# webster-781/DyGLib

Hardware: AMD Instinct MI355X
Metric: edges/sec (link-prediction fwd) DyGFormer Wikipedia (higher is better)
Workload: dtype f32; 1 GPU; DyGFormer link-prediction forward, synthetic wikipedia-shaped graph (8227+1000 nodes, 157474 edges), L=64, P=2, batch=200, 2 layers, 2 heads, C=50; pos+neg calls + MergeLayer+sigmoid per step; batch=200, max_input_sequence_length=64, patch_size=2, parallelism=1 x edge-batch shard, graph+weights replicated, metric all-reduce over RCCL, impl=auto, streams=1, steps_per_launch=32

## Files before the change

### dyglib_amd/_build.py

```python
from __future__ import annotations

import concurrent.futures as cf
import hashlib
import os
import shutil
import subprocess
import sys
from typing import List

CSRC = os.path.join(os.path.dirname(os.path.abspath(__file__)), "csrc")
INCLUDE = os.path.join(os.path.dirname(os.path.dirname(os.path.abspath(__file__))), "include")
LIB_NAME = "libdygnn_hip.so"
LIB_PATH = os.path.join(CSRC, LIB_NAME)
SOURCES = ["csr_host.cpp", "sampler.hip", "cooccurrence.hip", "dygformer_generic.hip", "dygformer_fused3.hip", "dygformer_fused3_train.hip",
           "dygformer_fused3_bwd.hip", "dygformer_fused3_pack.hip", "dygformer_pack_plan.hip", "dygformer_pooled_tail.hip", "dygformer_proj_tables.hip", "dygformer_train.hip",
           "dygformer_api.hip", "gemm.hip", "tgat.hip", "tgat_chain.hip", "tgat_train.hip", "tgn.hip", "tgn_train.hip", "graphmixer.hip", "graphmixer_train.hip", "tcl.hip", "tcl_train.hip", "cawn.hip",
           "cawn_train.hip", "metrics.hip", "edgebank.hip", "memory_rnn.hip"]
ARCH = "gfx950"
CXXFLAGS = ["-O3", "-std=c++17", "-fPIC", f"--offload-arch={ARCH}", "-Wall", "-Wno-unused-function",
            "-ffp-contract=off"]


SANITIZE = ["-fsanitize=address,undefined", "-fno-omit-frame-pointer", "-g", "-shared-libsan", "-Wno-option-ignored"]
VARIANTS = {"": [], "stamps": ["-DDYGNN_STAMPS=1"], "asan": SANITIZE}
for _k, _v in list(os.environ.items()):
    if _k.startswith("DYGNN_VARIANT_"):
        VARIANTS[_k[len("DYGNN_VARIANT_"):].lower()] = _v.split()
LINK_EXTRA = {"asan": ["-fsanitize=address,undefined", "-shared-libsan"]}


def asan_runtime() -> str:
    import glob
    hits = glob.glob("/opt/rocm/lib/llvm/lib/clang/*/lib/linux/libclang_rt.asan-x86_64.so")
    if not hits:
        raise RuntimeError("libclang_rt.asan-x86_64.so not found under /opt/rocm/lib/llvm")
    return hits[0]


def lib_path(variant: str = "") -> str:
    return LIB_PATH if not variant else os.path.join(CSRC, f"libdygnn_hip_{variant}.so")


def _hipcc() -> str:
    for cand in (os.environ.get("HIPCC"), "/opt/rocm/bin/hipcc", shutil.which("hipcc")):
        if cand and os.path.exists(cand):
            return cand
    raise RuntimeError("hipcc not found (looked at $HIPCC, /opt/rocm/bin/hipcc, PATH)")

# ... 67 lines not shown
```

### dyglib_amd/csrc/common.h

```cpp
#pragma once
#include <hip/hip_runtime.h>
#include <cstdarg>
#include <cstdint>
#include <cstdio>

#include "../../include/dygnn.h"

namespace dygnn {

void set_error(const char* fmt, ...);

inline hipStream_t as_stream(dygnn_stream_t s) { return reinterpret_cast<hipStream_t>(s); }

constexpr int kWave = 64;

inline int64_t ceil_div(int64_t a, int64_t b) { return (a + b - 1) / b; }

struct Carve {
    size_t o = 0;
    size_t take(size_t bytes) { const size_t r = o; o += (bytes + 255) & ~size_t(255); return r; }
};

__device__ __forceinline__ int64_t wave_lower_bound(const double* __restrict__ ts, int64_t lo, int64_t hi, double t, int lane) {
    while (hi - lo > kWave) {
        const int64_t step = (hi - lo + kWave - 1) / kWave;
        const int64_t p = lo + (int64_t)lane * step;
        const bool pred = (p < hi) && (ts[p] < t);
        const int c = __popcll(__ballot(pred));
        if (c == 0) return lo;
        const int64_t nlo = lo + (int64_t)(c - 1) * step + 1;
        const int64_t nhi = lo + (int64_t)c * step;
        hi = nhi < hi ? nhi : hi;
        lo = nlo;
    }
    const int64_t p = lo + lane;
    const bool pred = (p < hi) && (ts[p] < t);
    return lo + __popcll(__ballot(pred));
}

}

#define DYGNN_REQUIRE(cond, ...)                                  \
    do {                                                          \
        if (!(cond)) {                                            \
            dygnn::set_error(__VA_ARGS__);                        \
            return DYGNN_E_INVALID;                               \
        }                                                         \
    } while (0)

#define DYGNN_HIP(expr)                                                                        \
    do {                                                                                       \
        hipError_t _e = (expr);                                                                \
        if (_e != hipSuccess) {                                                                \
            dygnn::set_error("%s failed: %s (%s:%d)", #expr, hipGetErrorString(_e), __FILE__, __LINE__); \
            return DYGNN_E_HIP;                                                                \
        }                                                                                      \
    } while (0)

#define DYGNN_LAUNCH_CHECK() DYGNN_HIP(hipGetLastError())
```

### dyglib_amd/csrc/dygformer_fused3.hip

```cpp
#include "fused3_forward.h"

namespace dygnn {

namespace v3 {
__global__ __launch_bounds__(512, 2) void k_dygformer_fused3_packed(const Args a) {
    fused3_body<4, false, 8, 3, true>(a);
}
}

static void drop_zero_channels(v3::Args& a, uint32_t table_flags) {
    using namespace v3;
    const int node_frags = 4 * proj_slots(a.nchunk[0]), time_frags = 4 * proj_slots(a.nchunk[2]), edge_frags = 4 * proj_slots(a.nchunk[1]);
    if (table_flags & DYGNN_TABLE_NODE_ZERO) { a.proj_skip0 = node_frags; a.proj_frags -= node_frags; a.nchunk[0] = 0; }
    a.proj_cut = (a.nchunk[0] ? node_frags : 0) + time_frags;
    if (table_flags & DYGNN_TABLE_EDGE_ZERO) { a.proj_skip1 = edge_frags; a.proj_frags -= edge_frags; a.nchunk[1] = 0; }
}

int forward_fused3(const Dims& d, const PackedLayout& pl, const dygnn_dygformer_weights* w, const float* packed,
                   const dygnn_csr* csr, const float* node_feat, const float* edge_feat, const int64_t* src,
                   const int64_t* dst, const double* times, int64_t B, int64_t G, int64_t pair_stride, float* out_src, float* out_dst, char* ws,
                   const WorkspaceLayout& wl, const dygnn_dygformer_taps* taps, uint32_t table_flags, const float* node_proj, const float* edge_proj,
                   hipStream_t s) {
    using namespace v3;
    if (!supported(d)) { set_error("fused kernel: unsupported shape"); return DYGNN_E_UNSUPPORTED; }
    if (int rc = window_lengths_device(d, csr, src, dst, times, B, G, ws, wl, s)) return rc;
    Args a{};
    PackLayout3 f;
    if (int rc = fused3_args(d, pl, w, packed, csr, node_feat, edge_feat, src, dst, times, B, G, out_src, out_dst, ws, wl, taps, a, f)) return rc;
    if (table_flags & DYGNN_TABLE_NODE_ZERO) node_proj = nullptr;
    if (table_flags & DYGNN_TABLE_EDGE_ZERO) edge_proj = nullptr;
    drop_zero_channels(a, table_flags | (node_proj ? DYGNN_TABLE_NODE_ZERO : 0u) | (edge_proj ? DYGNN_TABLE_EDGE_ZERO : 0u));
    a.pt_node = node_proj; a.pt_edge = edge_proj;
    if (taps && taps->seq_lens) DYGNN_HIP(hipMemcpyAsync(taps->seq_lens, ws + wl.dims + 2 * sizeof(int32_t), 2 * sizeof(int32_t), hipMemcpyDeviceToDevice, s));
    if (taps && taps->ev_kernel_start) DYGNN_HIP(hipEventRecord(static_cast<hipEvent_t>(taps->ev_kernel_start), s));
    a.pair_stride = (f.np == 2 && pair_stride > 0) ? pair_stride : 0;
    const bool tap_last = taps && taps->layer_out[d.NL - 1] != nullptr;
    if (!tap_last) { a.stream = packed + pl.fused3 + f.stream_p; a.nstages = f.nstages_p; }
    bool untapped = !tap_last && !(taps && (taps->encoder_input || taps->phase_cycles));
    for (int l = 0; l < d.NL; ++l) untapped = untapped && !(taps && taps->layer_out[l]);
    const int pk_env = pack_pairs_env();
    const size_t plan_off = plan_offset(B, G);
    const bool pack_ok = untapped && f.np == 2 && f.scr_floats8 > 0 && B <= INT32_MAX && plan_off > 0 && pk_env != 0;
    const bool small = f.np == 2 && a.pair_stride == 0 && B <= kSmallBatchPairs && !small_off() && !(pack_ok && pk_env == 1);
    const unsigned grid = small || f.np != 2 ? (unsigned)B : (unsigned)(a.pair_stride ? a.pair_stride : (B + 1) / 2);
    auto launch = [&](auto kern, unsigned threads) -> int {
        DYGNN_HIP(hipFuncSetAttribute(reinterpret_cast<const void*>(kern), hipFuncAttributeMaxDynamicSharedMemorySize, kLdsBytes));
        hipLaunchKernelGGL(kern, dim3(grid), dim3(threads), kLdsBytes, s, a);
        return DYGNN_OK;
    };
    const bool tail = !tap_last && (pooled_tail_wanted(grid) || (pack_ok && pk_env == 1));
    const bool pack_it = pack_ok && !small && tail;
    int rc;
    if (pack_it) {
        if (int rcp = pack_plan_device(d, B, G, ws, wl, s)) return rcp;
        a.plan = reinterpret_cast<const int32_t*>(ws + wl.dims + plan_off);
        a.pair_stride = 0; a.scr_floats = f.scr_floats8; a.slab_chunks = f.slab_chunks8; a.tab_off = 0; a.tab_slots = 0; a.tab_bits = 0;
        rc = launch(k_dygformer_fused3_packed, 512);
    } else if (tail) rc = small ? launch(k_dygformer_fused3<4, false, 4, 3>, 256) : f.np == 2 ? launch(k_dygformer_fused3<4, false, 8, 3>, 512) : launch(k_dygformer_fused3<8, false, 8, 3>, 512);
    else if (small) rc = tap_last ? launch(k_dygformer_fused3<4, false, 4, 2>, 256) : launch(k_dygformer_fused3<4, false, 4, 1>, 256);
    else if (f.np == 2) rc = tap_last ? launch(k_dygformer_fused3<4, false, 8, 2>, 512) : launch(k_dygformer_fused3<4, false, 8, 1>, 512);
    else rc = tap_last ? launch(k_dygformer_fused3<8, false, 8, 2>, 512) : launch(k_dygformer_fused3<8, false, 8, 1>, 512);
    if (rc) return rc;
    DYGNN_LAUNCH_CHECK();
    if (tail)
        if (int rc2 = pooled_tail(a.pooled_rows, 2 * B, a.w2frag, a.b2_last, a.outfrag, a.outb, a.Fn, out_src, out_dst, s)) return rc2;
    if (taps && taps->ev_kernel_stop) DYGNN_HIP(hipEventRecord(static_cast<hipEvent_t>(taps->ev_kernel_stop), s));
    return DYGNN_OK;
}

}
```

### dyglib_amd/csrc/dygformer_pack_plan.hip

```cpp
#include "dygformer_layout.h"
#include "fused3_plan.h"

namespace dygnn {
namespace v3 {

constexpr int kPlanThreads = 1024;

__device__ __forceinline__ int pair_tile_count(const int32_t* hist_len, const CallDims* cd, int64_t b, int64_t B, int64_t G, int L, int P) {
    const CallDims d = cd[b / G];
    const PairTokens t = pair_tokens(hist_len[b], hist_len[B + b], L, P, d.T_s, d.T_d);
    const int nt = (t.Tc + 15) / 16;
    return nt < 1 ? 1 : nt > 4 ? 4 : nt;
}

__global__ __launch_bounds__(kPlanThreads) void k_pack_plan(const int32_t* hist_len, const CallDims* cd, int64_t B, int64_t G, int L, int P, int32_t* plan,
                                                            int32_t max_wg) {
    __shared__ int32_t cnt[2][4][kPlanThreads];
    __shared__ PackPlan pp;
    const int t = threadIdx.x;
    const int64_t chunk = (B + kPlanThreads - 1) / kPlanThreads;
    const int64_t b0 = t * chunk, b1 = b0 + chunk < B ? b0 + chunk : B;
    int32_t mine[4] = {0, 0, 0, 0};
    for (int64_t b = b0; b < b1; ++b) ++mine[pair_tile_count(hist_len, cd, b, B, G, L, P) - 1];
    for (int k = 0; k < 4; ++k) cnt[0][k][t] = mine[k];
    __syncthreads();
    int cur = 0;
    for (int off = 1; off < kPlanThreads; off <<= 1) {
        for (int k = 0; k < 4; ++k) cnt[cur ^ 1][k][t] = cnt[cur][k][t] + (t >= off ? cnt[cur][k][t - off] : 0);
        cur ^= 1;
        __syncthreads();
    }
    if (t == 0) {
        pp = make_pack_plan(cnt[cur][0][kPlanThreads - 1], cnt[cur][1][kPlanThreads - 1], cnt[cur][2][kPlanThreads - 1], cnt[cur][3][kPlanThreads - 1]);
    }
    __syncthreads();
    const bool fits = pp.used <= max_wg;
    int32_t* ent = plan;
    for (int64_t i = t; i < (int64_t)max_wg * 8; i += kPlanThreads) ent[i] = -1;
    __syncthreads();
    int32_t rank[4];
    for (int k = 0; k < 4; ++k) rank[k] = cnt[cur][k][t] - mine[k];
    for (int64_t b = b0; b < b1 && fits; ++b) {
        const int nt = pair_tile_count(hist_len, cd, b, B, G, L, P);
        const PlanSlot sl = plan_slot(pp, nt, rank[nt - 1]++);
        for (int w = 0; w < nt; ++w) ent[(int64_t)sl.wg * 8 + sl.fw + w] = (int32_t)b;
    }
}

}

int pack_plan_device(const Dims& d, int64_t B, int64_t G, char* ws, const WorkspaceLayout& wl, hipStream_t s) {
    using namespace v3;
    hipLaunchKernelGGL(k_pack_plan, dim3(1), dim3(kPlanThreads), 0, s, reinterpret_cast<const int32_t*>(ws + wl.hist_len),
                       reinterpret_cast<const CallDims*>(ws + wl.dims), B, G, d.L, d.P, reinterpret_cast<int32_t*>(ws + wl.dims + plan_offset(B, G)),
                       (int32_t)((B + 1) / 2));
    DYGNN_LAUNCH_CHECK();
    return DYGNN_OK;
}

}

extern "C" int64_t dygnn_dygformer_pack_plan_host(const int32_t* tiles, int64_t n, int32_t* wg, int32_t* fw) {
    using namespace dygnn::v3;
    int64_t cnt[5] = {0, 0, 0, 0, 0};
    for (int64_t i = 0; i < n; ++i) {
        if (tiles[i] < 1 || tiles[i] > 4) return -1;
        ++cnt[tiles[i]];
    }
    const PackPlan pp = make_pack_plan(cnt[1], cnt[2], cnt[3], cnt[4]);
    int32_t rank[5] = {0, 0, 0, 0, 0};
    for (int64_t i = 0; i < n; ++i) {
        const PlanSlot sl = plan_slot(pp, tiles[i], rank[tiles[i]]++);
        wg[i] = sl.wg; fw[i] = sl.fw;
    }
    return pp.used;
}
extern "C" void dygnn_dygformer_pair_tokens_host(int32_t len_s, int32_t len_d, int32_t L, int32_t P, int32_t T_s, int32_t T_d, int32_t* out) {
    const dygnn::v3::PairTokens t = dygnn::v3::pair_tokens(len_s, len_d, L, P, T_s, T_d);
    out[0] = t.Rs; out[1] = t.Rd; out[2] = t.ms; out[3] = t.md; out[4] = t.Tc;
// ... 2 lines not shown
```

### dyglib_amd/csrc/fused3_device.h

```cpp
#pragma once
#include "dygformer_layout.h"


namespace dygnn {
namespace v3 {

using f4 = __attribute__((ext_vector_type(4))) float;
using i4 = __attribute__((ext_vector_type(4))) int;

constexpr int kD = 200, kDP = 208, kNT = 13, kKC = 13, kHD = 100, kHid = 800, kC = 50;
constexpr int kFrag = 256;
constexpr int kPoolRow = kHid + kDP;
constexpr int kRing = 52;
constexpr int kStage = 13;
constexpr int kNStage = kRing / kStage;
static_assert(kStage * kNStage == kRing && kNStage >= 2, "the ring is a whole number (>= 2) of stages");
constexpr int kTokWG = 128;
constexpr int kKV = 100;
constexpr int kLdsK = 0;
constexpr int kLdsV = kTokWG * kKV;
constexpr int kLdsRing = 2 * kTokWG * kKV + 16;
constexpr int kLdsMisc = kLdsRing + kRing * kFrag;
constexpr int kMiscB1 = 0;
constexpr int kMiscFloats = 2 * kHid;
// ... 12 lines not shown
    for (int u = 0; u < N; ++u) acc[u] = mfma(a[u].z, b.z, acc[u]);
#pragma unroll
    for (int u = 0; u < N; ++u) acc[u] = mfma(a[u].w, b.w, acc[u]);
}
template <int N>
__device__ __forceinline__ void mma_group2(f4* acc, const f4* a, const float b0, const float b1) {
#pragma unroll
    for (int u = 0; u < N; ++u) acc[u] = mfma(a[u].x, b0, acc[u]);
#pragma unroll
    for (int u = 0; u < N; ++u) acc[u] = mfma(a[u].y, b1, acc[u]);
}
__device__ __forceinline__ void kpack(const f4 v, float& b0, float& b1) {
    const float vx = v.x, vy = v.y, vz = v.z, vw = v.w;
    const auto r0 = __builtin_amdgcn_permlane32_swap(__builtin_bit_cast(unsigned, vx), __builtin_bit_cast(unsigned, vy), false, false);
    const auto r1 = __builtin_amdgcn_permlane32_swap(__builtin_bit_cast(unsigned, vz), __builtin_bit_cast(unsigned, vw), false, false);
    b0 = __builtin_bit_cast(float, r0[0]);
    b1 = __builtin_bit_cast(float, r1[0]);
}
__device__ __forceinline__ float kpack4(const f4 v) {
    const float vx = v.x, vy = v.y, vz = v.z, vw = v.w;
    const auto t1 = __builtin_amdgcn_permlane16_swap(__builtin_bit_cast(unsigned, vx), __builtin_bit_cast(unsigned, vy), false, false);
    const auto t2 = __builtin_amdgcn_permlane16_swap(__builtin_bit_cast(unsigned, vz), __builtin_bit_cast(unsigned, vw), false, false);
    const auto r = __builtin_amdgcn_permlane32_swap(t1[0], t2[0], false, false);
    return __builtin_bit_cast(float, r[0]);
}
template <int N>
__device__ __forceinline__ void mma_group1(f4* acc, const f4* a, const float b0) {
#pragma unroll
    for (int u = 0; u < N; ++u) acc[u] = mfma(a[u].x, b0, acc[u]);
}
__device__ __forceinline__ f4 ldg4(const float* p) { return *reinterpret_cast<const f4*>(p); }
__device__ __forceinline__ f4 lds4(const float* p) { return *reinterpret_cast<const f4*>(p); }
__device__ __forceinline__ f4 zero4() { return f4{0.f, 0.f, 0.f, 0.f}; }
#pragma clang diagnostic push
#pragma clang diagnostic ignored "-Winline-asm"
__device__ __forceinline__ void dma_frag(const float* gsrc_lane, int lds_float_off_uniform) {
    const unsigned m0v = __builtin_amdgcn_readfirstlane(__builtin_amdgcn_groupstaticsize() + 4u * (unsigned)lds_float_off_uniform);
    asm volatile("s_mov_b32 m0, %1\n\ts_nop 0\n\tglobal_load_lds_dwordx4 %0, off" ::"v"(gsrc_lane), "s"(m0v) : "memory", "m0");
}
#pragma clang diagnostic pop

template <int CTRL>
__device__ __forceinline__ float dpp_mov(float v) {
    return __builtin_bit_cast(float, __builtin_amdgcn_update_dpp(0, __builtin_bit_cast(int, v), CTRL, 0xF, 0xF, true));
}
__device__ __forceinline__ float row_sum16(float v) {
    v += dpp_mov<0xB1>(v);
    v += dpp_mov<0x4E>(v);
    v += dpp_mov<0x141>(v);
    v += dpp_mov<0x140>(v);
    return v;
}
__device__ __forceinline__ float keep_scalar(float v) { asm("" : "+v"(v)); return v; }
__device__ __forceinline__ float row_sum16_dpp(float v) {
    v = keep_scalar(v + dpp_mov<0xB1>(v));
    v = keep_scalar(v + dpp_mov<0x4E>(v));
    v = keep_scalar(v + dpp_mov<0x141>(v));
    v = keep_scalar(v + dpp_mov<0x140>(v));
    return v;
}

__device__ __forceinline__ float cos_time_fast(float x) {
    const float INV_HI = 0.15915493667125702f, INV_LO = 6.4206382432985265e-09f;
    const float p = x * INV_HI;
    const float e = fmaf(x, INV_HI, -p);
    const float q = fmaf(x, INV_LO, e);
// ... 132 lines not shown
    for (int i = 0; i < kNT; ++i) {
        if (i < 12 || g < 2) {
            const float d0 = x[i].x - mean, d1 = x[i].y - mean, d2 = x[i].z - mean, d3 = x[i].w - mean;
            v += (d0 * d0 + d1 * d1) + (d2 * d2 + d3 * d3);
        }
    }
    v += __shfl_xor(v, 16, 64);
    v += __shfl_xor(v, 32, 64);
    const float rstd = 1.0f / sqrtf(v * (1.0f / kD) + 1e-5f);
    mean_o = mean; rstd_o = rstd;
#pragma unroll
    for (int i = 0; i < kNT; ++i) {
        const f4 gm = lds4(gamma + 16 * i + 4 * g), bt = lds4(beta + 16 * i + 4 * g);
        xn[i].x = (x[i].x - mean) * rstd * gm.x + bt.x;
        xn[i].y = (x[i].y - mean) * rstd * gm.y + bt.y;
        xn[i].z = (x[i].z - mean) * rstd * gm.z + bt.z;
        xn[i].w = (x[i].w - mean) * rstd * gm.w + bt.w;
    }
}

template <int NT>
__device__ __forceinline__ void qkv_group(f4 (&acc)[NT], const f4 (&xn)[kNT], const float xk0, const float xk1, WStream& ws, const float* ringl, bool active) {
    constexpr int N2 = NT - 4;
    f4 fs[2][4];
    ws.fit(NT);
    if (active) {
#pragma unroll
        for (int u = 0; u < 4; ++u) fs[0][u] = lds4(ringl + (ws.pos + u) * kFrag);
    }
#pragma unroll
    for (int kc = 0; kc < kKC; ++kc) {
        if (active) {
#pragma unroll
            for (int u = 0; u < N2; ++u) fs[1][u] = lds4(ringl + (ws.pos + 4 + u) * kFrag);
            __builtin_amdgcn_sched_barrier(0);
            if (kc == kKC - 1) mma_group2<4>(&acc[0], fs[0], xk0, xk1); else mma_group<4>(&acc[0], fs[0], xn[kc]);
            __builtin_amdgcn_sched_barrier(0);
            if (kc + 1 < kKC) {
                const int p1 = ws.next_pos(NT, NT);
#pragma unroll
                for (int u = 0; u < 4; ++u) fs[0][u] = lds4(ringl + (p1 + u) * kFrag);
            }
            __builtin_amdgcn_sched_barrier(0);
            if (kc == kKC - 1) mma_group2<N2>(&acc[4], fs[1], xk0, xk1); else mma_group<N2>(&acc[4], fs[1], xn[kc]);
            __builtin_amdgcn_sched_barrier(0);
        }
        ws.advance(NT);
        if (kc + 1 < kKC) ws.fit(NT);
    }
}

__device__ __forceinline__ void ffn_w1(f4 (&h)[2], const f4 (&xn)[kNT], const float xk0, const float xk1, const float* abuf, const float* b1p, const int g) {
    if (b1p != nullptr) { h[0] = lds4(b1p + 4 * g); h[1] = lds4(b1p + 16 + 4 * g); }
    else { h[0] = zero4(); h[1] = zero4(); }
    f4 sa[2][2];
    sa[0][0] = lds4(abuf); sa[0][1] = lds4(abuf + kFrag);
#pragma unroll
    for (int kc = 0; kc < kKC; ++kc) {
        const int cur = kc & 1;
        if (kc + 1 < kKC) {
            sa[cur ^ 1][0] = lds4(abuf + (size_t)(2 * (kc + 1)) * kFrag);
            sa[cur ^ 1][1] = lds4(abuf + (size_t)(2 * (kc + 1) + 1) * kFrag);
        }
        __builtin_amdgcn_sched_barrier(0);
        if (kc == kKC - 1) mma_group2<2>(h, sa[cur], xk0, xk1); else mma_group<2>(h, sa[cur], xn[kc]);
        __builtin_amdgcn_sched_barrier(0);
    }
}
__device__ __forceinline__ void ffn_w2(f4 (&acc)[kNT], const f4 (&h)[2], const float* bbuf) {
    f4 fs[2][4];
#pragma unroll
    for (int v = 0; v < 4; ++v) fs[0][v] = lds4(bbuf + (size_t)v * kFrag);
#pragma unroll
    for (int gi = 0; gi < 8; ++gi) {
        const int u = gi >> 2, q = gi & 3;
        const int i0 = q == 0 ? 0 : 4 + 3 * (q - 1), n = q == 0 ? 4 : 3;
        if (gi + 1 < 8) {
            const int u2 = (gi + 1) >> 2, q2 = (gi + 1) & 3;
            const int j0 = q2 == 0 ? 0 : 4 + 3 * (q2 - 1), n2 = q2 == 0 ? 4 : 3;
#pragma unroll
            for (int v = 0; v < 4; ++v) if (v < n2) fs[(gi + 1) & 1][v] = lds4(bbuf + (size_t)(u2 * 13 + j0 + v) * kFrag);
        }
        __builtin_amdgcn_sched_barrier(0);
        if (n == 4) mma_group<4>(&acc[i0], fs[gi & 1], h[u]); else mma_group<3>(&acc[i0], fs[gi & 1], h[u]);
        __builtin_amdgcn_sched_barrier(0);
    }
}

template <int TPW>
__device__ __forceinline__ void s_like(f4 (&sa)[TPW], const float* base, const f4 (&q)[7], int c, int g) {
    const float q6 = kpack4(q[6]);
#pragma unroll
    for (int kh = 0; kh < TPW / 4; ++kh) {
        const float* kbase = base + (64 * kh + c) * kKV + 4 * g;
        f4 kf[2][4];
// ... 49 lines not shown
    };
    f4 va[2][4];
    load_v(va[0], 0, 0, 4);
#pragma unroll
    for (int st = 0; st < 2 * TPW; ++st) {
        const int kt = st >> 1, half = st & 1;
        if (st + 1 < 2 * TPW) load_v(va[(st + 1) & 1], (st + 1) >> 1, ((st + 1) & 1) ? 4 : 0, ((st + 1) & 1) ? 3 : 4);
        __builtin_amdgcn_sched_barrier(0);
        if (half == 0) mma_group<4>(&oa[0], va[st & 1], p[kt]); else mma_group<3>(&oa[4], va[st & 1], p[kt]);
        __builtin_amdgcn_sched_barrier(0);
    }
}
__device__ __forceinline__ void proj_t(f4 (&acc)[kNT], const f4 (&t)[7], WStream& ws, const float* ringl, bool active) {
    ws.fit(13);
    f4 fs[2][4];
    float t6 = 0.f;
    if (active) {
#pragma unroll
        for (int v = 0; v < 4; ++v) fs[0][v] = lds4(ringl + (ws.pos + v) * kFrag);
        t6 = kpack4(t[6]);
    }
#pragma unroll
    for (int j = 0; j < 7; ++j) {
        const int pcur = ws.pos;
        const int pnext = ws.next_pos(13, 13);
        if (active) {
#pragma unroll
            for (int q = 0; q < 4; ++q) {
                const int gi = 4 * j + q;
                const int i0 = q == 0 ? 0 : 4 + 3 * (q - 1), n = q == 0 ? 4 : 3;
                if (q + 1 < 4) {
                    const int j0 = 4 + 3 * q;
#pragma unroll
                    for (int v = 0; v < 3; ++v) fs[(gi + 1) & 1][v] = lds4(ringl + (pcur + j0 + v) * kFrag);
                } else if (j + 1 < 7) {
#pragma unroll
                    for (int v = 0; v < 4; ++v) fs[(gi + 1) & 1][v] = lds4(ringl + (pnext + v) * kFrag);
                }
                __builtin_amdgcn_sched_barrier(0);
                if (j == 6) { if (n == 4) mma_group1<4>(&acc[i0], fs[gi & 1], t6); else mma_group1<3>(&acc[i0], fs[gi & 1], t6); }
                else if (n == 4) mma_group<4>(&acc[i0], fs[gi & 1], t[j]); else mma_group<3>(&acc[i0], fs[gi & 1], t[j]);
                __builtin_amdgcn_sched_barrier(0);
            }
        }
        ws.advance(13);
        if (j + 1 < 7) ws.fit(13);
    }
}
}
}
```

### dyglib_amd/csrc/fused3_forward.h

```cpp
#pragma once
#include <type_traits>

#include "dropout.h"
#include "fused3_device.h"
#include "fused3_host.h"
#include "fused3_plan.h"

namespace dygnn {
namespace v3 {

struct LayerP {
    const float* b1;
};

struct Args {
    const int64_t* indptr; const int32_t* nbr; const int32_t* eid; const double* ts;
    const int64_t *src, *dst; const double* times;
    const int32_t* hist_len; const int64_t* end_pos; const CallDims* cd;
    const float *node_feat, *edge_feat, *time_w, *time_b, *lut;
    const float* stream; int nstages;
    const float* projw;
    int proj_frags;
    int proj_skip0, proj_cut, proj_skip1;
    int slab_chunks;
// ... 367 lines not shown
        };

        struct TCur { int pp, f; float dt; bool ok; int32_t idn; float dn; f4 w, bb; };
        auto tpos_at = [&](int pp, float& dt, bool& ok) {
            const int q = pos0 + (pp < P ? pp : P - 1);
            const int32_t id = ids[q];
            const float d = dts[q];
            ok = tv && pp < P && id > 0;
            dt = ok ? d : 0.f;
        };
        auto t_advance = [&](TCur& tc) {
            tc.f += 16;
            const bool wrap = tc.f >= a.Ft;
            tc.f = wrap ? tc.f - a.Ft : tc.f;
            const bool okn = tv && tc.pp + 1 < P && tc.idn > 0;
            tc.dt = wrap ? (okn ? tc.dn : 0.f) : tc.dt;
            tc.ok = wrap ? okn : tc.ok;
            tc.pp += wrap ? 1 : 0;
            const int q = pos0 + (tc.pp + 1 < P ? tc.pp + 1 : P - 1);
            tc.idn = ids[q];
            tc.dn = dts[q];
            tc.w = lds4(tws + tc.f);
            tc.bb = lds4(tws + a.Ft + tc.f);
        };
        auto t_finish = [&](const bool ok, const f4 arg, f4 cs) -> f4 {
            if (!(fabsf(arg.x) <= 3.0e7f && fabsf(arg.y) <= 3.0e7f && fabsf(arg.z) <= 3.0e7f && fabsf(arg.w) <= 3.0e7f)) {
                cs.x = cos_time(arg.x); cs.y = cos_time(arg.y); cs.z = cos_time(arg.z); cs.w = cos_time(arg.w);
            }
            return ok ? cs : zero4();
        };
        auto t_group = [&](auto L0c, auto NSc, auto FRESHc, f4 (&fa)[2][4], f4& bnx, TCur& tc) {
            constexpr int L0 = decltype(L0c)::value, NS = decltype(NSc)::value;
            const float* fr = frag_ptr();
            if (decltype(FRESHc)::value) read_frags(fa[0], fr);
#pragma unroll
            for (int u = 0; u < NS; ++u) {
                const f4 bcur = bnx;
                const f4 w = tc.w, bb = tc.bb;
                frags_ahead(NSc, u, fr, fa, false);
                __builtin_amdgcn_sched_barrier(0);
                const f2 dt2 = {tc.dt, tc.dt};
                const f2 a01 = pk_fma(dt2, f2{w.x, w.y}, f2{bb.x, bb.y}), a23 = pk_fma(dt2, f2{w.z, w.w}, f2{bb.z, bb.w});
                const f2 c01 = cos_time_fast2(a01), c23 = cos_time_fast2(a23);
                const f4 arg = {a01.x, a01.y, a23.x, a23.y}, cs = {c01.x, c01.y, c23.x, c23.y};
                const bool okc = tc.ok;
                t_advance(tc);
                mma_group<4>(&x[L0], fa[u & 1], bcur);
                __builtin_amdgcn_sched_barrier(0);
                bnx = t_finish(okc, arg, cs);
            }
        };
        auto run_time = [&](auto L0c, int n) {
            f4 fa[2][4];
            TCur tc{0, 4 * g, 0.f, false, 0, 0.f, zero4(), zero4()};
            tpos_at(0, tc.dt, tc.ok);
            { const int q = pos0 + (1 < P ? 1 : P - 1); tc.idn = ids[q]; tc.dn = dts[q]; }
            f4 bnx;
            {
                const f4 w = lds4(tws + tc.f), bb = lds4(tws + a.Ft + tc.f);
                f4 arg;
                arg.x = fmaf(tc.dt, w.x, bb.x); arg.y = fmaf(tc.dt, w.y, bb.y); arg.z = fmaf(tc.dt, w.z, bb.z); arg.w = fmaf(tc.dt, w.w, bb.w);
                f4 cs;
                cs.x = cos_time_fast(arg.x); cs.y = cos_time_fast(arg.y); cs.z = cos_time_fast(arg.z); cs.w = cos_time_fast(arg.w);
                bnx = t_finish(tc.ok, arg, cs);
                t_advance(tc);
            }
            const int ng = n / GS, rem = n % GS;
// ... 551 lines not shown
```

### dyglib_amd/csrc/fused3_host.h

```cpp
#pragma once
#include <cstdlib>

#include "common.h"

namespace dygnn {

struct Dims;
struct PackedLayout;
struct WorkspaceLayout;
namespace train { struct Drop; struct TrainOut; }

namespace v3 {

struct PackLayout3 {
    size_t bias_x;
    size_t stream; int64_t nfrag; int nstages;
    size_t aux; int64_t naux;
    size_t proj; int64_t nproj;
    int scr_floats, slab_chunks;
    int np, slab_in_ring;
    int tab_off, tab_slots, tab_bits;
    int scr_floats8, slab_chunks8;
    size_t bwd[DYGNN_MAX_LAYERS]; int bwd_nstages;
    size_t bwa[DYGNN_MAX_LAYERS]; int bwa_nstages; int64_t bwa_frags;
    size_t stream_p; int64_t nfrag_p; int nstages_p;
    size_t w2;
    size_t desc;
    size_t total;
};

PackLayout3 make_layout3(const Dims& d);
bool supported(const Dims& d);
int proj_slots(int nchunk);

}

constexpr int64_t kSmallBatchPairs = 256;
inline bool small_off() { static const bool off = [] { const char* e = getenv("DYGNN_SMALL_BATCH_KERNELS"); return e && e[0] == '0'; }(); return off; }

constexpr int64_t kPooledTailMinWorkgroups = 2000;
inline bool pooled_tail_wanted(int64_t workgroups) {
    const char* e = getenv("DYGNN_POOLED_TAIL");
    if (e && (e[0] == '0' || e[0] == '1') && e[1] == '\0') return e[0] == '1';
    return workgroups >= kPooledTailMinWorkgroups;
}

inline int pack_pairs_env() {
    const char* e = getenv("DYGNN_PACK_PAIRS");
    return (e && (e[0] == '0' || e[0] == '1') && e[1] == '\0') ? e[0] - '0' : -1;
}
int pack_plan_device(const Dims& d, int64_t B, int64_t G, char* ws, const WorkspaceLayout& wl, hipStream_t s);

constexpr int kProjRow = 64;
inline bool proj_tables_off() { const char* e = getenv("DYGNN_PROJ_TABLES"); return e && e[0] == '0' && e[1] == '\0'; }

int window_lengths_device(const Dims& d, const dygnn_csr* csr, const int64_t* src, const int64_t* dst, const double* times,
                          int64_t B, int64_t G, char* ws, const WorkspaceLayout& wl, hipStream_t s);
bool fused3_supported(const Dims& d);
size_t fused3_packed_floats(const Dims& d);
int pack_fused3(const Dims& d, const PackedLayout& pl, const dygnn_dygformer_weights* w, float* packed, hipStream_t s, bool reuse_desc);
int forward_fused3(const Dims& d, const PackedLayout& pl, const dygnn_dygformer_weights* w, const float* packed,
                   const dygnn_csr* csr, const float* node_feat, const float* edge_feat, const int64_t* src,
                   const int64_t* dst, const double* times, int64_t B, int64_t G, int64_t pair_stride, float* out_src, float* out_dst, char* ws,
                   const WorkspaceLayout& wl, const dygnn_dygformer_taps* taps, uint32_t table_flags, const float* node_proj, const float* edge_proj,
                   hipStream_t s);
int pooled_tail(const float* rows, int64_t R, const float* w2frag, const float* b2, const float* outfrag, const float* outb, int Fn,
                float* out_src, float* out_dst, hipStream_t s);
int forward_fused3_train(const Dims& d, const PackedLayout& pl, const dygnn_dygformer_weights* w, const float* packed, const dygnn_csr* csr,
                         const float* node_feat, const float* edge_feat, const int64_t* src, const int64_t* dst, const double* times, int64_t B,
                         const float* lut, float* out_src, float* out_dst, char* ws, const WorkspaceLayout& wl, const train::TrainOut& tr, hipStream_t s);
int ffn_backward_fused3(const Dims& d, const PackedLayout& pl, const float* packed, int l, int64_t M, float* dX, const float* hpre, const float* x1,
                        const float* m1, const float* r1, float* dF2, float* dH, float* dgamma, float* dbeta, const train::Drop& dr, hipStream_t s);
int attn_backward_fused3(const Dims& d, const PackedLayout& pl, const float* packed, int l, int64_t B, int T, float* dX, const float* X, const float* m0,
                         const float* r0, const float* qkv, const float* P, const float* Pd, float* dAo, float* dQKV, float* dgamma, float* dbeta,
                         const train::Drop& dr, hipStream_t s);

}
```

### dyglib_amd/csrc/sampler.hip

```cpp
#include "common.h"

namespace dygnn {

struct CsrView {
    const int64_t* indptr;
    const int32_t* nbr;
    const int32_t* eid;
    const double* ts;
    int64_t num_nodes;
};

__device__ __forceinline__ void query_row(const CsrView& g, int64_t node, int64_t& row_lo, int64_t& row_hi) {
    if (node < 0 || node >= g.num_nodes) node = 0;
    row_lo = g.indptr[node];
    row_hi = g.indptr[node + 1];
}

__global__ __launch_bounds__(256) void k_find_before(CsrView g, const int64_t* __restrict__ nodes,
                                                       const double* __restrict__ times, int64_t n, int32_t clampL,
                                                       int32_t* __restrict__ hist_len, int64_t* __restrict__ end_pos,
                                                       int32_t* __restrict__ max_window) {
    const int lane = threadIdx.x & 63;
    const int64_t q = (int64_t)blockIdx.x * (blockDim.x >> 6) + (threadIdx.x >> 6);
    if (q >= n) return;
// ... 7 lines not shown
        if (max_window) {
            const int32_t v = len < clampL ? len : clampL;
            if (v > __atomic_load_n(max_window, __ATOMIC_RELAXED)) atomicMax(max_window, v);
        }
    }
}

__global__ __launch_bounds__(256) void k_sample_recent(CsrView g, const int64_t* __restrict__ nodes,
                                                         const double* __restrict__ times, int64_t n, int32_t k,
                                                         int64_t* __restrict__ out_nbr, int64_t* __restrict__ out_eid,
                                                         float* __restrict__ out_ts) {
    const int lane = threadIdx.x & 63;
    const int64_t q = (int64_t)blockIdx.x * (blockDim.x >> 6) + (threadIdx.x >> 6);
    if (q >= n) return;
    int64_t lo, hi;
    query_row(g, nodes[q], lo, hi);
    const int64_t i = wave_lower_bound(g.ts, lo, hi, times[q], lane);
    const int64_t len = i - lo;
    const int32_t m = (int32_t)(len < k ? len : k);
    const int32_t pad = k - m;
    int64_t* on = out_nbr + q * k;
    int64_t* oe = out_eid + q * k;
    float* ot = out_ts + q * k;
    for (int32_t j = lane; j < k; j += kWave) {
        if (j < pad) {
            on[j] = 0; oe[j] = 0; ot[j] = 0.0f;
        } else {
            const int64_t p = i - m + (j - pad);
            on[j] = g.nbr[p]; oe[j] = g.eid[p]; ot[j] = (float)g.ts[p];
        }
    }
}

constexpr int kSub = 16;

__device__ __forceinline__ int64_t sub_lower_bound(const double* __restrict__ ts, int64_t lo, int64_t hi, double t, int sl, int sg) {
    while (__any(hi - lo > kSub)) {
        const bool wide = hi - lo > kSub;
        const int64_t step = wide ? (hi - lo + kSub - 1) / kSub : 1;
        const int64_t p = lo + (int64_t)sl * step;
        const bool pred = wide && (p < hi) && (ts[p] < t);
        const int c = __popc((unsigned)((__ballot(pred) >> (kSub * sg)) & 0xFFFFull));
        if (wide) {
            if (c == 0) hi = lo;
            else {
                const int64_t nlo = lo + (int64_t)(c - 1) * step + 1, nhi = lo + (int64_t)c * step;
                hi = nhi < hi ? nhi : hi;
                lo = nlo;
            }
        }
    }
    const int64_t p = lo + sl;
    const bool pred = (p < hi) && (ts[p] < t);
    return lo + __popc((unsigned)((__ballot(pred) >> (kSub * sg)) & 0xFFFFull));
}

__global__ __launch_bounds__(256) void k_sample_recent_sub(CsrView g, const int64_t* __restrict__ nodes, const double* __restrict__ times, int64_t n,
                                                             int32_t k, int64_t* __restrict__ out_nbr, int64_t* __restrict__ out_eid,
                                                             float* __restrict__ out_ts) {
    const int lane = threadIdx.x & 63, sg = lane / kSub, sl = lane % kSub;
    const int64_t q = ((int64_t)blockIdx.x * (blockDim.x >> 6) + (threadIdx.x >> 6)) * (kWave / kSub) + sg;
    const bool on = q < n;
    int64_t lo = 0, hi = 0;
    double t = 0.0;
    if (on) { query_row(g, nodes[q], lo, hi); t = times[q]; }
    const int64_t i = sub_lower_bound(g.ts, lo, hi, t, sl, sg);
    if (!on) return;
    const int64_t len = i - lo;
    const int32_t m = (int32_t)(len < k ? len : k);
    const int32_t pad = k - m;
    int64_t* on_ = out_nbr + q * k;
    int64_t* oe = out_eid + q * k;
    float* ot = out_ts + q * k;
    for (int32_t j = sl; j < k; j += kSub) {
        if (j < pad) {
            on_[j] = 0; oe[j] = 0; ot[j] = 0.0f;
        } else {
            const int64_t p = i - m + (j - pad);
            on_[j] = g.nbr[p]; oe[j] = g.eid[p]; ot[j] = (float)g.ts[p];
        }
    }
}

__global__ __launch_bounds__(256) void k_find_before_sub(CsrView g, const int64_t* __restrict__ nodes, const double* __restrict__ times, int64_t n,
                                                           int32_t clampL, int32_t* __restrict__ hist_len, int64_t* __restrict__ end_pos,
                                                           int32_t* __restrict__ max_window) {
    const int lane = threadIdx.x & 63, sg = lane / kSub, sl = lane % kSub;
    const int64_t q = ((int64_t)blockIdx.x * (blockDim.x >> 6) + (threadIdx.x >> 6)) * (kWave / kSub) + sg;
// ... 154 lines not shown
```

Measured before the change: 557,100 edges/s.

## Fuse window-length search, call-dims reduction and pack plan into one setup kernel

Replaces the separate window-length kernels and the pack-plan kernel with a single setup kernel. It runs the sub-wave binary search, then uses a last-block ticket to compute per-group call dims and, when packing is used, builds the pack plan in the same launch. This is meant to cut launch count and inter-kernel gaps in a small-batch forward. It also narrows LDS fragment reads on the final K chunk and adds an explicit waitcnt before fresh fragment reads. The grid-wide ticket relies on threadfence ordering, and the last block does the serial plan work alone.

```diff
diff --git a/dyglib_amd/_build.py b/dyglib_amd/_build.py
--- a/dyglib_amd/_build.py
+++ b/dyglib_amd/_build.py
@@ -13,7 +13,7 @@
 LIB_NAME = "libdygnn_hip.so"
 LIB_PATH = os.path.join(CSRC, LIB_NAME)
 SOURCES = ["csr_host.cpp", "sampler.hip", "cooccurrence.hip", "dygformer_generic.hip", "dygformer_fused3.hip", "dygformer_fused3_train.hip",
-           "dygformer_fused3_bwd.hip", "dygformer_fused3_pack.hip", "dygformer_pack_plan.hip", "dygformer_pooled_tail.hip", "dygformer_proj_tables.hip", "dygformer_train.hip",
+           "dygformer_fused3_bwd.hip", "dygformer_fused3_pack.hip", "dygformer_pack_plan.hip", "dygformer_setup.hip", "dygformer_pooled_tail.hip", "dygformer_proj_tables.hip", "dygformer_train.hip",
            "dygformer_api.hip", "gemm.hip", "tgat.hip", "tgat_chain.hip", "tgat_train.hip", "tgn.hip", "tgn_train.hip", "graphmixer.hip", "graphmixer_train.hip", "tcl.hip", "tcl_train.hip", "cawn.hip",
            "cawn_train.hip", "metrics.hip", "edgebank.hip", "memory_rnn.hip"]
 ARCH = "gfx950"
diff --git a/dyglib_amd/csrc/common.h b/dyglib_amd/csrc/common.h
--- a/dyglib_amd/csrc/common.h
+++ b/dyglib_amd/csrc/common.h
@@ -38,6 +38,28 @@
     return lo + __popcll(__ballot(pred));
 }
 
+constexpr int kSub = 16;
+__device__ __forceinline__ int64_t sub_lower_bound(const double* __restrict__ ts, int64_t lo, int64_t hi, double t, int sl, int sg) {
+    while (__any(hi - lo > kSub)) {
+        const bool wide = hi - lo > kSub;
+        const int64_t step = wide ? (hi - lo + kSub - 1) / kSub : 1;
+        const int64_t p = lo + (int64_t)sl * step;
+        const bool pred = wide && (p < hi) && (ts[p] < t);
+        const int c = __popc((unsigned)((__ballot(pred) >> (kSub * sg)) & 0xFFFFull));
+        if (wide) {
+            if (c == 0) hi = lo;
+            else {
+                const int64_t nlo = lo + (int64_t)(c - 1) * step + 1, nhi = lo + (int64_t)c * step;
+                hi = nhi < hi ? nhi : hi;
+                lo = nlo;
+            }
+        }
+    }
+    const int64_t p = lo + sl;
+    const bool pred = (p < hi) && (ts[p] < t);
+    return lo + __popc((unsigned)((__ballot(pred) >> (kSub * sg)) & 0xFFFFull));
+}
+
 }
 
 #define DYGNN_REQUIRE(cond, ...)                                  \
diff --git a/dyglib_amd/csrc/dygformer_fused3.hip b/dyglib_amd/csrc/dygformer_fused3.hip
--- a/dyglib_amd/csrc/dygformer_fused3.hip
+++ b/dyglib_amd/csrc/dygformer_fused3.hip
@@ -23,7 +23,6 @@
                    hipStream_t s) {
     using namespace v3;
     if (!supported(d)) { set_error("fused kernel: unsupported shape"); return DYGNN_E_UNSUPPORTED; }
-    if (int rc = window_lengths_device(d, csr, src, dst, times, B, G, ws, wl, s)) return rc;
     Args a{};
     PackLayout3 f;
     if (int rc = fused3_args(d, pl, w, packed, csr, node_feat, edge_feat, src, dst, times, B, G, out_src, out_dst, ws, wl, taps, a, f)) return rc;
@@ -31,8 +30,6 @@
     if (table_flags & DYGNN_TABLE_EDGE_ZERO) edge_proj = nullptr;
     drop_zero_channels(a, table_flags | (node_proj ? DYGNN_TABLE_NODE_ZERO : 0u) | (edge_proj ? DYGNN_TABLE_EDGE_ZERO : 0u));
     a.pt_node = node_proj; a.pt_edge = edge_proj;
-    if (taps && taps->seq_lens) DYGNN_HIP(hipMemcpyAsync(taps->seq_lens, ws + wl.dims + 2 * sizeof(int32_t), 2 * sizeof(int32_t), hipMemcpyDeviceToDevice, s));
-    if (taps && taps->ev_kernel_start) DYGNN_HIP(hipEventRecord(static_cast<hipEvent_t>(taps->ev_kernel_start), s));
     a.pair_stride = (f.np == 2 && pair_stride > 0) ? pair_stride : 0;
     const bool tap_last = taps && taps->layer_out[d.NL - 1] != nullptr;
     if (!tap_last) { a.stream = packed + pl.fused3 + f.stream_p; a.nstages = f.nstages_p; }
@@ -50,9 +47,14 @@
     };
     const bool tail = !tap_last && (pooled_tail_wanted(grid) || (pack_ok && pk_env == 1));
     const bool pack_it = pack_ok && !small && tail;
+    const bool plan_in_setup = pack_it && pooled_tail_wanted(grid);
+    if (int rcs = launch_setup_device(d, csr, src, dst, times, B, G, ws, wl, plan_in_setup, s)) return rcs;
+    if (taps && taps->seq_lens) DYGNN_HIP(hipMemcpyAsync(taps->seq_lens, ws + wl.dims + 2 * sizeof(int32_t), 2 * sizeof(int32_t), hipMemcpyDeviceToDevice, s));
+    if (taps && taps->ev_kernel_start) DYGNN_HIP(hipEventRecord(static_cast<hipEvent_t>(taps->ev_kernel_start), s));
     int rc;
     if (pack_it) {
-        if (int rcp = pack_plan_device(d, B, G, ws, wl, s)) return rcp;
+        if (!plan_in_setup)
+            if (int rcp = pack_plan_device(d, B, G, ws, wl, s)) return rcp;
         a.plan = reinterpret_cast<const int32_t*>(ws + wl.dims + plan_off);
         a.pair_stride = 0; a.scr_floats = f.scr_floats8; a.slab_chunks = f.slab_chunks8; a.tab_off = 0; a.tab_slots = 0; a.tab_bits = 0;
         rc = launch(k_dygformer_fused3_packed, 512);
diff --git a/dyglib_amd/csrc/dygformer_pack_plan.hip b/dyglib_amd/csrc/dygformer_pack_plan.hip
--- a/dyglib_amd/csrc/dygformer_pack_plan.hip
+++ b/dyglib_amd/csrc/dygformer_pack_plan.hip
@@ -1,50 +1,12 @@
-#include "dygformer_layout.h"
-#include "fused3_plan.h"
+#include "fused3_plan_device.h"
 
 namespace dygnn {
 namespace v3 {
 
-constexpr int kPlanThreads = 1024;
-
-__device__ __forceinline__ int pair_tile_count(const int32_t* hist_len, const CallDims* cd, int64_t b, int64_t B, int64_t G, int L, int P) {
-    const CallDims d = cd[b / G];
-    const PairTokens t = pair_tokens(hist_len[b], hist_len[B + b], L, P, d.T_s, d.T_d);
-    const int nt = (t.Tc + 15) / 16;
-    return nt < 1 ? 1 : nt > 4 ? 4 : nt;
-}
-
 __global__ __launch_bounds__(kPlanThreads) void k_pack_plan(const int32_t* hist_len, const CallDims* cd, int64_t B, int64_t G, int L, int P, int32_t* plan,
                                                             int32_t max_wg) {
-    __shared__ int32_t cnt[2][4][kPlanThreads];
-    __shared__ PackPlan pp;
-    const int t = threadIdx.x;
-    const int64_t chunk = (B + kPlanThreads - 1) / kPlanThreads;
-    const int64_t b0 = t * chunk, b1 = b0 + chunk < B ? b0 + chunk : B;
-    int32_t mine[4] = {0, 0, 0, 0};
-    for (int64_t b = b0; b < b1; ++b) ++mine[pair_tile_count(hist_len, cd, b, B, G, L, P) - 1];
-    for (int k = 0; k < 4; ++k) cnt[0][k][t] = mine[k];
-    __syncthreads();
-    int cur = 0;
-    for (int off = 1; off < kPlanThreads; off <<= 1) {
-        for (int k = 0; k < 4; ++k) cnt[cur ^ 1][k][t] = cnt[cur][k][t] + (t >= off ? cnt[cur][k][t - off] : 0);
-        cur ^= 1;
-        __syncthreads();
-    }
-    if (t == 0) {
-        pp = make_pack_plan(cnt[cur][0][kPlanThreads - 1], cnt[cur][1][kPlanThreads - 1], cnt[cur][2][kPlanThreads - 1], cnt[cur][3][kPlanThreads - 1]);
-    }
-    __syncthreads();
-    const bool fits = pp.used <= max_wg;
-    int32_t* ent = plan;
-    for (int64_t i = t; i < (int64_t)max_wg * 8; i += kPlanThreads) ent[i] = -1;
-    __syncthreads();
-    int32_t rank[4];
-    for (int k = 0; k < 4; ++k) rank[k] = cnt[cur][k][t] - mine[k];
-    for (int64_t b = b0; b < b1 && fits; ++b) {
-        const int nt = pair_tile_count(hist_len, cd, b, B, G, L, P);
-        const PlanSlot sl = plan_slot(pp, nt, rank[nt - 1]++);
-        for (int w = 0; w < nt; ++w) ent[(int64_t)sl.wg * 8 + sl.fw + w] = (int32_t)b;
-    }
+    __shared__ PlanShared sh;
+    pack_plan_block(sh, hist_len, cd, B, G, L, P, plan, max_wg);
 }
 
 }
diff --git a/dyglib_amd/csrc/dygformer_setup.hip b/dyglib_amd/csrc/dygformer_setup.hip
--- /dev/null
+++ b/dyglib_amd/csrc/dygformer_setup.hip
@@ -0,0 +1,134 @@
+#include "fused3_plan_device.h"
+
+namespace dygnn {
+namespace v3 {
+
+constexpr int kSetupThreads = kPlanThreads;
+constexpr int kSetupWaves = kSetupThreads / kWave;
+constexpr int kSetupQueries = kSetupThreads / kSub;
+
+struct SetupArgs {
+    const int64_t* indptr; const double* ts; int64_t num_nodes;
+    const int64_t *src, *dst; const double* times;
+    int64_t B, G;
+    int32_t L, P;
+    int32_t* hist_len; int64_t* end_pos; CallDims* cd;
+    unsigned* ticket;
+    int32_t* plan; int32_t max_wg;
+};
+
+__device__ __forceinline__ int32_t wave_max_i32(int32_t v) {
+#pragma unroll
+    for (int o = 32; o > 0; o >>= 1) { const int32_t u = __shfl_xor(v, o, 64); v = u > v ? u : v; }
+    return v;
+}
+
+__device__ __forceinline__ void write_call_dims(CallDims* cd, int32_t maxw_s, int32_t maxw_d, int P) {
+    int Ss = maxw_s + 1, Sd = maxw_d + 1;
+    if (Ss % P) Ss += P - Ss % P;
+    if (Sd % P) Sd += P - Sd % P;
+    cd->maxw_s = maxw_s; cd->maxw_d = maxw_d; cd->S_s = Ss; cd->S_d = Sd; cd->T_s = Ss / P; cd->T_d = Sd / P; cd->T = Ss / P + Sd / P;
+}
+
+__global__ __launch_bounds__(kSetupThreads) void k_launch_setup(const SetupArgs a) {
+    __shared__ PlanShared sh;
+    __shared__ int32_t wmax[2][kSetupWaves];
+    __shared__ int is_last;
+    const int t = threadIdx.x, wave = t >> 6, lane = t & 63, sg = lane / kSub, sl = lane % kSub;
+    const int64_t B = a.B, G = a.G;
+    const int64_t q = ((int64_t)blockIdx.x * kSetupWaves + wave) * (kWave / kSub) + sg;
+    const bool on = q < 2 * B;
+    int64_t lo = 0, hi = 0;
+    double tq = 0.0;
+    if (on) {
+        const bool is_dst = q >= B;
+        const int64_t r = is_dst ? q - B : q;
+        int64_t node = is_dst ? a.dst[r] : a.src[r];
+        if (node < 0 || node >= a.num_nodes) node = 0;
+        lo = a.indptr[node]; hi = a.indptr[node + 1];
+        tq = a.times[r];
+    }
+    const int64_t row_lo = lo;
+    const int64_t i = sub_lower_bound(a.ts, lo, hi, tq, sl, sg);
+    if (on && sl == 0) {
+        a.hist_len[q] = (int32_t)(i - row_lo);
+        a.end_pos[q] = i;
+    }
+    asm volatile("s_waitcnt vmcnt(0)" ::: "memory");
+    __syncthreads();
+    if (t == 0) {
+        __threadfence();
+        asm volatile("s_waitcnt vmcnt(0)" ::: "memory");
+        is_last = atomicAdd(a.ticket, 1u) == gridDim.x - 1;
+        if (is_last) __threadfence();
+    }
+    __syncthreads();
+    if (!is_last) return;
+
+    const int64_t ng = (B + G - 1) / G;
+    const int32_t cap = a.L - 1;
+    auto win = [&](int64_t qi) { const int32_t len = a.hist_len[qi]; return len < cap ? len : cap; };
+    if (ng < kSetupWaves) {
+        for (int64_t gi = 0; gi < ng; ++gi) {
+            const int64_t b0 = gi * G, b1 = b0 + G < B ? b0 + G : B;
+            int32_t ms = 0, md = 0;
+            for (int64_t b = b0 + t; b < b1; b += kSetupThreads) { const int32_t vs = win(b), vd = win(B + b); ms = vs > ms ? vs : ms; md = vd > md ? vd : md; }
+            ms = wave_max_i32(ms); md = wave_max_i32(md);
+            if (lane == 0) { wmax[0][wave] = ms; wmax[1][wave] = md; }
+            __syncthreads();
+            if (t == 0) {
+                for (int w = 1; w < kSetupWaves; ++w) { ms = wmax[0][w] > ms ? wmax[0][w] : ms; md = wmax[1][w] > md ? wmax[1][w] : md; }
+                write_call_dims(a.cd + gi, ms, md, a.P);
+            }
+            __syncthreads();
+        }
+    } else if (G >= kSub) {
+        for (int64_t gi = wave; gi < ng; gi += kSetupWaves) {
+            const int64_t b0 = gi * G, b1 = b0 + G < B ? b0 + G : B;
+            int32_t ms = 0, md = 0;
+            for (int64_t b = b0 + lane; b < b1; b += kWave) { const int32_t vs = win(b), vd = win(B + b); ms = vs > ms ? vs : ms; md = vd > md ? vd : md; }
+            ms = wave_max_i32(ms); md = wave_max_i32(md);
+            if (lane == 0) write_call_dims(a.cd + gi, ms, md, a.P);
+        }
+    } else {
+        for (int64_t gi = t; gi < ng; gi += kSetupThreads) {
+            const int64_t b0 = gi * G, b1 = b0 + G < B ? b0 + G : B;
+            int32_t ms = 0, md = 0;
+            for (int64_t b = b0; b < b1; ++b) { const int32_t vs = win(b), vd = win(B + b); ms = vs > ms ? vs : ms; md = vd > md ? vd : md; }
+            write_call_dims(a.cd + gi, ms, md, a.P);
+        }
+    }
+    if (a.plan != nullptr) {
+        asm volatile("s_waitcnt vmcnt(0)" ::: "memory");
+        __syncthreads();
+        if (t == 0) __threadfence();
+        __syncthreads();
+        pack_plan_block(sh, a.hist_len, a.cd, B, G, a.L, a.P, a.plan, a.max_wg);
+    }
+    if (t == 0) *a.ticket = 0u;
+}
+
+}
+
+int launch_setup_device(const Dims& d, const dygnn_csr* csr, const int64_t* src, const int64_t* dst, const double* times, int64_t B, int64_t G,
+                        char* ws, const WorkspaceLayout& wl, bool with_plan, hipStream_t s) {
+    using namespace v3;
+    DYGNN_REQUIRE(2 * B <= (int64_t)INT32_MAX * kSetupQueries, "launch set-up: batch too large");
+    SetupArgs a{};
+    a.indptr = csr->indptr; a.ts = csr->ts; a.num_nodes = csr->num_nodes;
+    a.src = src; a.dst = dst; a.times = times; a.B = B; a.G = G; a.L = d.L; a.P = d.P;
+    a.hist_len = reinterpret_cast<int32_t*>(ws + wl.hist_len);
+    a.end_pos = reinterpret_cast<int64_t*>(ws + wl.end_pos);
+    a.cd = reinterpret_cast<CallDims*>(ws + wl.dims);
+    a.ticket = reinterpret_cast<unsigned*>(&a.cd->pad);
+    if (with_plan) {
+        a.plan = reinterpret_cast<int32_t*>(ws + wl.dims + plan_offset(B, G));
+        a.max_wg = (int32_t)((B + 1) / 2);
+    }
+    DYGNN_HIP(hipMemsetAsync(a.cd, 0, sizeof(CallDims), s));
+    hipLaunchKernelGGL(k_launch_setup, dim3((unsigned)ceil_div(2 * B, kSetupQueries)), dim3(kSetupThreads), 0, s, a);
+    DYGNN_LAUNCH_CHECK();
+    return DYGNN_OK;
+}
+
+}
diff --git a/dyglib_amd/csrc/fused3_device.h b/dyglib_amd/csrc/fused3_device.h
--- a/dyglib_amd/csrc/fused3_device.h
+++ b/dyglib_amd/csrc/fused3_device.h
@@ -68,6 +68,15 @@
 __device__ __forceinline__ f4 ldg4(const float* p) { return *reinterpret_cast<const f4*>(p); }
 __device__ __forceinline__ f4 lds4(const float* p) { return *reinterpret_cast<const f4*>(p); }
 __device__ __forceinline__ f4 zero4() { return f4{0.f, 0.f, 0.f, 0.f}; }
+using f2 = __attribute__((ext_vector_type(2))) float;
+__device__ __forceinline__ void lds_frag2(f4& d, const float* p, bool last) {
+    if (last) { const f2 v = *reinterpret_cast<const f2*>(p); d.x = v.x; d.y = v.y; }
+    else d = lds4(p);
+}
+__device__ __forceinline__ void lds_frag1(f4& d, const float* p, bool last) {
+    if (last) d.x = *p;
+    else d = lds4(p);
+}
 #pragma clang diagnostic push
 #pragma clang diagnostic ignored "-Winline-asm"
 __device__ __forceinline__ void dma_frag(const float* gsrc_lane, int lds_float_off_uniform) {
@@ -266,14 +275,14 @@
     for (int kc = 0; kc < kKC; ++kc) {
         if (active) {
 #pragma unroll
-            for (int u = 0; u < N2; ++u) fs[1][u] = lds4(ringl + (ws.pos + 4 + u) * kFrag);
+            for (int u = 0; u < N2; ++u) lds_frag2(fs[1][u], ringl + (ws.pos + 4 + u) * kFrag, kc == kKC - 1);
             __builtin_amdgcn_sched_barrier(0);
             if (kc == kKC - 1) mma_group2<4>(&acc[0], fs[0], xk0, xk1); else mma_group<4>(&acc[0], fs[0], xn[kc]);
             __builtin_amdgcn_sched_barrier(0);
             if (kc + 1 < kKC) {
                 const int p1 = ws.next_pos(NT, NT);
 #pragma unroll
-                for (int u = 0; u < 4; ++u) fs[0][u] = lds4(ringl + (p1 + u) * kFrag);
+                for (int u = 0; u < 4; ++u) lds_frag2(fs[0][u], ringl + (p1 + u) * kFrag, kc + 1 == kKC - 1);
             }
             __builtin_amdgcn_sched_barrier(0);
             if (kc == kKC - 1) mma_group2<N2>(&acc[4], fs[1], xk0, xk1); else mma_group<N2>(&acc[4], fs[1], xn[kc]);
@@ -293,8 +302,8 @@
     for (int kc = 0; kc < kKC; ++kc) {
         const int cur = kc & 1;
         if (kc + 1 < kKC) {
-            sa[cur ^ 1][0] = lds4(abuf + (size_t)(2 * (kc + 1)) * kFrag);
-            sa[cur ^ 1][1] = lds4(abuf + (size_t)(2 * (kc + 1) + 1) * kFrag);
+            lds_frag2(sa[cur ^ 1][0], abuf + (size_t)(2 * (kc + 1)) * kFrag, kc + 1 == kKC - 1);
+            lds_frag2(sa[cur ^ 1][1], abuf + (size_t)(2 * (kc + 1) + 1) * kFrag, kc + 1 == kKC - 1);
         }
         __builtin_amdgcn_sched_barrier(0);
         if (kc == kKC - 1) mma_group2<2>(h, sa[cur], xk0, xk1); else mma_group<2>(h, sa[cur], xn[kc]);
@@ -410,10 +419,10 @@
                 if (q + 1 < 4) {
                     const int j0 = 4 + 3 * q;
 #pragma unroll
-                    for (int v = 0; v < 3; ++v) fs[(gi + 1) & 1][v] = lds4(ringl + (pcur + j0 + v) * kFrag);
+                    for (int v = 0; v < 3; ++v) lds_frag1(fs[(gi + 1) & 1][v], ringl + (pcur + j0 + v) * kFrag, j == 6);
                 } else if (j + 1 < 7) {
 #pragma unroll
-                    for (int v = 0; v < 4; ++v) fs[(gi + 1) & 1][v] = lds4(ringl + (pnext + v) * kFrag);
+                    for (int v = 0; v < 4; ++v) lds_frag1(fs[(gi + 1) & 1][v], ringl + (pnext + v) * kFrag, j + 1 == 6);
                 }
                 __builtin_amdgcn_sched_barrier(0);
                 if (j == 6) { if (n == 4) mma_group1<4>(&acc[i0], fs[gi & 1], t6); else mma_group1<3>(&acc[i0], fs[gi & 1], t6); }
diff --git a/dyglib_amd/csrc/fused3_forward.h b/dyglib_amd/csrc/fused3_forward.h
--- a/dyglib_amd/csrc/fused3_forward.h
+++ b/dyglib_amd/csrc/fused3_forward.h
@@ -423,7 +423,10 @@
         auto t_group = [&](auto L0c, auto NSc, auto FRESHc, f4 (&fa)[2][4], f4& bnx, TCur& tc) {
             constexpr int L0 = decltype(L0c)::value, NS = decltype(NSc)::value;
             const float* fr = frag_ptr();
-            if (decltype(FRESHc)::value) read_frags(fa[0], fr);
+            if (decltype(FRESHc)::value) {
+                if constexpr (!TR) __builtin_amdgcn_s_waitcnt(0xc07f);
+                read_frags(fa[0], fr);
+            }
 #pragma unroll
             for (int u = 0; u < NS; ++u) {
                 const f4 bcur = bnx;
diff --git a/dyglib_amd/csrc/fused3_host.h b/dyglib_amd/csrc/fused3_host.h
--- a/dyglib_amd/csrc/fused3_host.h
+++ b/dyglib_amd/csrc/fused3_host.h
@@ -51,6 +51,9 @@
 }
 int pack_plan_device(const Dims& d, int64_t B, int64_t G, char* ws, const WorkspaceLayout& wl, hipStream_t s);
 
+int launch_setup_device(const Dims& d, const dygnn_csr* csr, const int64_t* src, const int64_t* dst, const double* times, int64_t B, int64_t G,
+                        char* ws, const WorkspaceLayout& wl, bool with_plan, hipStream_t s);
+
 constexpr int kProjRow = 64;
 inline bool proj_tables_off() { const char* e = getenv("DYGNN_PROJ_TABLES"); return e && e[0] == '0' && e[1] == '\0'; }
 
diff --git a/dyglib_amd/csrc/fused3_plan_device.h b/dyglib_amd/csrc/fused3_plan_device.h
--- /dev/null
+++ b/dyglib_amd/csrc/fused3_plan_device.h
@@ -0,0 +1,67 @@
+#pragma once
+#include "dygformer_layout.h"
+#include "fused3_plan.h"
+
+namespace dygnn {
+namespace v3 {
+
+constexpr int kPlanThreads = 1024;
+
+struct PlanShared {
+    int32_t cnt[2][4][kPlanThreads];
+    PackPlan pp;
+};
+
+__device__ __forceinline__ void pack_plan_block(PlanShared& sh, const int32_t* hist_len, const CallDims* cd, int64_t B, int64_t G, int L, int P, int32_t* plan,
+                                                int32_t max_wg) {
+    const int t = threadIdx.x;
+    const int64_t chunk = (B + kPlanThreads - 1) / kPlanThreads;
+    const int64_t b0 = t * chunk, b1 = b0 + chunk < B ? b0 + chunk : B;
+    auto run_tiles = [&](auto&& f) {
+        if (b0 >= b1) return;
+        int64_t gi = b0 / G, gend = (gi + 1) * G;
+        CallDims d = cd[gi];
+        for (int64_t b = b0; b < b1; ++b) {
+            if (b == gend) { ++gi; gend += G; d = cd[gi]; }
+            const PairTokens t = pair_tokens(hist_len[b], hist_len[B + b], L, P, d.T_s, d.T_d);
+            const int nt = (t.Tc + 15) / 16;
+            f(b, nt < 1 ? 1 : nt > 4 ? 4 : nt);
+        }
+    };
+    int32_t mine[4] = {0, 0, 0, 0};
+    uint64_t kept = 0;
+    run_tiles([&](int64_t b, int nt) {
+        ++mine[nt - 1];
+        if (b - b0 < 32) kept |= (uint64_t)(nt - 1) << (2 * (b - b0));
+    });
+    for (int k = 0; k < 4; ++k) sh.cnt[0][k][t] = mine[k];
+    __syncthreads();
+    int cur = 0;
+    for (int off = 1; off < kPlanThreads; off <<= 1) {
+        for (int k = 0; k < 4; ++k) sh.cnt[cur ^ 1][k][t] = sh.cnt[cur][k][t] + (t >= off ? sh.cnt[cur][k][t - off] : 0);
+        cur ^= 1;
+        __syncthreads();
+    }
+    if (t == 0) {
+        sh.pp = make_pack_plan(sh.cnt[cur][0][kPlanThreads - 1], sh.cnt[cur][1][kPlanThreads - 1], sh.cnt[cur][2][kPlanThreads - 1],
+                               sh.cnt[cur][3][kPlanThreads - 1]);
+    }
+    __syncthreads();
+    const bool fits = sh.pp.used <= max_wg;
+    int32_t* ent = plan;
+    for (int64_t i = t; i < (int64_t)max_wg * 8; i += kPlanThreads) ent[i] = -1;
+    __syncthreads();
+    int32_t rank[4];
+    for (int k = 0; k < 4; ++k) rank[k] = sh.cnt[cur][k][t] - mine[k];
+    auto place = [&](int64_t b, int nt) {
+        const PlanSlot sl = plan_slot(sh.pp, nt, rank[nt - 1]++);
+        for (int w = 0; w < nt; ++w) ent[(int64_t)sl.wg * 8 + sl.fw + w] = (int32_t)b;
+    };
+    if (!fits) return;
+    if (b1 - b0 <= 32) {
+        for (int64_t b = b0; b < b1; ++b) place(b, (int)((kept >> (2 * (b - b0))) & 3) + 1);
+    } else run_tiles(place);
+}
+
+}
+}
diff --git a/dyglib_amd/csrc/sampler.hip b/dyglib_amd/csrc/sampler.hip
--- a/dyglib_amd/csrc/sampler.hip
+++ b/dyglib_amd/csrc/sampler.hip
@@ -63,28 +63,6 @@
     }
 }
 
-constexpr int kSub = 16;
-
-__device__ __forceinline__ int64_t sub_lower_bound(const double* __restrict__ ts, int64_t lo, int64_t hi, double t, int sl, int sg) {
-    while (__any(hi - lo > kSub)) {
-        const bool wide = hi - lo > kSub;
-        const int64_t step = wide ? (hi - lo + kSub - 1) / kSub : 1;
-        const int64_t p = lo + (int64_t)sl * step;
-        const bool pred = wide && (p < hi) && (ts[p] < t);
-        const int c = __popc((unsigned)((__ballot(pred) >> (kSub * sg)) & 0xFFFFull));
-        if (wide) {
-            if (c == 0) hi = lo;
-            else {
-                const int64_t nlo = lo + (int64_t)(c - 1) * step + 1, nhi = lo + (int64_t)c * step;
-                hi = nhi < hi ? nhi : hi;
-                lo = nlo;
-            }
-        }
-    }
-    const int64_t p = lo + sl;
-    const bool pred = (p < hi) && (ts[p] < t);
-    return lo + __popc((unsigned)((__ballot(pred) >> (kSub * sg)) & 0xFFFFull));
-}
 
 __global__ __launch_bounds__(256) void k_sample_recent_sub(CsrView g, const int64_t* __restrict__ nodes, const double* __restrict__ times, int64_t n,
                                                              int32_t k, int64_t* __restrict__ out_nbr, int64_t* __restrict__ out_eid,
```

Result: no change. 560,300 edges/s, median of 6 (+0.6%).
